# funcwj/setk

Hardware: AMD Instinct MI355X
Metric: real-time-factor (audio-sec/wall-sec), 8-ch 16 kHz MVDR (higher is better)
Workload: dtype f32; 1 GPU; 8-ch 16 kHz oracle-mask MVDR, 30 s utterances, 125 per GPU (BASELINE configs[2] shard: 1000 at 8 GPUs), STFT 512/256/hann/center, inputs resident in HBM; utts_per_gpu=125, channels=8, frames=1876, beamformer=mvdr, parallelism=utterance-sharded x1

## Files before the change

### setk_amd/csrc/mcdft.h

```cpp
#pragma once
#include <hip/hip_runtime.h>
#include <stdint.h>

namespace setk {
namespace mc {

#define MC_DEV __device__ __forceinline__

typedef _Float16 h8 __attribute__((ext_vector_type(8)));
typedef _Float16 h2 __attribute__((ext_vector_type(2)));
typedef float f4 __attribute__((ext_vector_type(4)));
typedef float f2 __attribute__((ext_vector_type(2)));
typedef unsigned u4 __attribute__((ext_vector_type(4)));

enum : int {
    kW_MC_H = 0, kW_MC_L = 4, kW_MS_H = 8, kW_MS_L = 12,
    kW_AR_H = 16, kW_AR_L = 20, kW_AI_H = 24, kW_AI_L = 28,
    kW_TR = 32, kW_TI = 36, kW_TRI = 40,
    kW_OT_H = 44, kW_OT_L = 48,
    kW_BR_H = 52, kW_BR_L = 56, kW_BI_H = 60, kW_BI_L = 64,
    kW_G0_H = 68, kW_G0_L = 72, kW_G1_H = 76, kW_G1_L = 80,
    kW_IT_H = 84, kW_IT_L = 88,
    kTabWords = 92
};

__host__ __device__ constexpr int stage1_n1(int k) {
    return (k % 8 < 4) ? 4 * (k / 8) + k % 8 : 16 + 4 * (k / 8) + k % 8 - 4;
}
__host__ __device__ constexpr int sample_of(int lane, int e) { return 16 * stage1_n1(8 * (lane >> 4) + e) + (lane & 15); }

MC_DEV h8 tab_h8(const unsigned* tab, int word, int lane) {
    u4 w;
    w[0] = tab[(word + 0) * 64 + lane];
    w[1] = tab[(word + 1) * 64 + lane];
    w[2] = tab[(word + 2) * 64 + lane];
    w[3] = tab[(word + 3) * 64 + lane];
    return __builtin_bit_cast(h8, w);
}
MC_DEV float tab_f(const unsigned* tab, int word, int lane) {
    return __builtin_bit_cast(float, tab[word * 64 + lane]);
}

MC_DEV f4 mfma16(h8 a, h8 b, f4 c) { return __builtin_amdgcn_mfma_f32_16x16x32_f16(a, b, c, 0, 0, 0); }

MC_DEV void sub_h2(float a, float b, h2 p, float& la, float& lb) {
    const unsigned w = __builtin_bit_cast(unsigned, p);
    asm("v_fma_mix_f32 %0, %1, 1.0, -%2 op_sel_hi:[0,0,1]" : "=v"(la) : "v"(a), "v"(w));
    asm("v_fma_mix_f32 %0, %1, 1.0, -%2 op_sel:[0,0,1] op_sel_hi:[0,0,1]" : "=v"(lb) : "v"(b), "v"(w));
}

MC_DEV void split8(const float (&v)[8], h8& hi, h8& lo) {
#pragma unroll
    for (int e = 0; e < 8; e += 2) {
        const h2 p = __builtin_convertvector((f2){v[e], v[e + 1]}, h2);
        hi[e] = p[0];
        hi[e + 1] = p[1];
        float la, lb;
        sub_h2(v[e], v[e + 1], p, la, lb);
        const h2 q = __builtin_convertvector((f2){la, lb}, h2);
        lo[e] = q[0];
        lo[e + 1] = q[1];
    }
}
MC_DEV void split8_hi(const float (&v)[8], h8& hi) {
#pragma unroll
    for (int e = 0; e < 8; e += 2) {
        const h2 p = __builtin_convertvector((f2){v[e], v[e + 1]}, h2);
        hi[e] = p[0];
        hi[e + 1] = p[1];
    }
}
MC_DEV void split8_lo(const float (&v)[8], h8 hi, h8& lo) {
#pragma unroll
    for (int e = 0; e < 8; e += 2) {
        float la, lb;
        sub_h2(v[e], v[e + 1], (h2){hi[e], hi[e + 1]}, la, lb);
        const h2 q = __builtin_convertvector((f2){la, lb}, h2);
        lo[e] = q[0];
        lo[e + 1] = q[1];
    }
}
MC_DEV void split8_mul_hi(const float (&v)[8], const float (&w)[8], h8& hi) {
#pragma unroll
    for (int e = 0; e < 8; e += 2) {
        const h2 p = __builtin_convertvector((f2){v[e] * w[e], v[e + 1] * w[e + 1]}, h2);
        hi[e] = p[0];
        hi[e + 1] = p[1];
    }
}
MC_DEV void split8_mul_lo(const float (&v)[8], const float (&w)[8], h8 hi, h8& lo) {
#pragma unroll
    for (int e = 0; e < 8; e += 2) {
        const h2 q = __builtin_convertvector(
            (f2){__builtin_fmaf(v[e], w[e], -(float)hi[e]), __builtin_fmaf(v[e + 1], w[e + 1], -(float)hi[e + 1])}, h2);
        lo[e] = q[0];
        lo[e + 1] = q[1];
    }
}
MC_DEV void split8_mul(const float (&v)[8], const float (&w)[8], h8& hi, h8& lo) {
#pragma unroll
    for (int e = 0; e < 8; e += 2) {
        const h2 p = __builtin_convertvector((f2){v[e] * w[e], v[e + 1] * w[e + 1]}, h2);
        hi[e] = p[0];
        hi[e + 1] = p[1];
        const h2 q = __builtin_convertvector(
            (f2){__builtin_fmaf(v[e], w[e], -(float)p[0]), __builtin_fmaf(v[e + 1], w[e + 1], -(float)p[1])}, h2);
        lo[e] = q[0];
        lo[e + 1] = q[1];
    }
}

MC_DEV f4 mm3_data_a(h8 dh, h8 dl, h8 kh, h8 kl) {
    f4 d = {0.f, 0.f, 0.f, 0.f};
    d = mfma16(dh, kh, d);
    d = mfma16(dl, kh, d);
    d = mfma16(dh, kl, d);
    return d;
}
MC_DEV f4 mm3_data_b(h8 kh, h8 kl, h8 dh, h8 dl) {
    f4 d = {0.f, 0.f, 0.f, 0.f};
    d = mfma16(kh, dh, d);
    d = mfma16(kh, dl, d);
    d = mfma16(kl, dh, d);
    return d;
}

struct Fwd {
    h8 mc_h, mc_l, ms_h, ms_l;
    h8 ar_h, ar_l, ai_h, ai_l;
    float tr[4], ti[4], tri[4];
};
MC_DEV void load_fwd(Fwd& K, const unsigned* tab, int lane) {
    K.mc_h = tab_h8(tab, kW_MC_H, lane);
    K.mc_l = tab_h8(tab, kW_MC_L, lane);
    K.ms_h = tab_h8(tab, kW_MS_H, lane);
    K.ms_l = tab_h8(tab, kW_MS_L, lane);
    K.ar_h = tab_h8(tab, kW_AR_H, lane);
    K.ar_l = tab_h8(tab, kW_AR_L, lane);
    K.ai_h = tab_h8(tab, kW_AI_H, lane);
    K.ai_l = tab_h8(tab, kW_AI_L, lane);
#pragma unroll
    for (int r = 0; r < 4; ++r) {
        K.tr[r] = tab_f(tab, kW_TR + r, lane);
        K.ti[r] = tab_f(tab, kW_TI + r, lane);
        K.tri[r] = tab_f(tab, kW_TRI + r, lane);
    }
}

template <class TileFn>
MC_DEV void forward_t(const float (&x)[8], const float (&w)[8], TileFn tile, const float (&tr)[4],
                      const float (&ti)[4], const float (&tri)[4], f4& zr, f4& zi, f4& a16) {
    h8 xh, xl;
    split8_mul_hi(x, w, xh);
    f4 dc = {0.f, 0.f, 0.f, 0.f}, ds = {0.f, 0.f, 0.f, 0.f};
    {
        const h8 mc_h = tile(0), ms_h = tile(2);
        dc = mfma16(xh, mc_h, dc);
        ds = mfma16(xh, ms_h, ds);
        dc = mfma16(xh, tile(1), dc);
        ds = mfma16(xh, tile(3), ds);
        split8_mul_lo(x, w, xh, xl);
        dc = mfma16(xl, mc_h, dc);
        ds = mfma16(xl, ms_h, ds);
    }
    a16 = ds;
    float b[8];
#pragma unroll
    for (int r = 0; r < 4; ++r) {
        b[r] = fmaf(dc[r], tr[r], -ds[r] * ti[r]);
        b[4 + r] = fmaf(dc[r], ti[r], ds[r] * tri[r]);
    }
    h8 bh, bl;
    split8_hi(b, bh);
    zr = (f4){0.f, 0.f, 0.f, 0.f};
    zi = (f4){0.f, 0.f, 0.f, 0.f};
    {
        const h8 ar_h = tile(4), ai_h = tile(6);
        zr = mfma16(ar_h, bh, zr);
        zi = mfma16(ai_h, bh, zi);
        zr = mfma16(tile(5), bh, zr);
        zi = mfma16(tile(7), bh, zi);
        split8_lo(b, bh, bl);
        zr = mfma16(ar_h, bl, zr);
        zi = mfma16(ai_h, bl, zi);
    }
}
MC_DEV void forward(const float (&x)[8], const float (&w)[8], const Fwd& K, f4& zr, f4& zi, f4& a16) {
    forward_t(x, w, [&](int i) -> h8 {
        switch (i) {
            case 0: return K.mc_h;
            case 1: return K.mc_l;
            case 2: return K.ms_h;
            case 3: return K.ms_l;
            case 4: return K.ar_h;
            case 5: return K.ar_l;
            case 6: return K.ai_h;
            default: return K.ai_l;
        }
    }, K.tr, K.ti, K.tri, zr, zi, a16);
}

MC_DEV int bin_of(int c, int g, int r) { return (g < 2) ? c + 32 * (4 * g + r) : 32 * (13 - 4 * g + r) - c; }
MC_DEV bool bin_valid(int c, int g, int r) { return c != 0 || g < 2 || (g == 2 && r == 3); }

typedef __attribute__((address_space(3))) float* lds_fp;
MC_DEV lds_fp to_lds(float* p) { return (lds_fp)p; }
MC_DEV lds_fp opaque_next(lds_fp p) {
    lds_fp q = p + 1;
    asm volatile("" : "+v"(q));
    return q;
}
MC_DEV void store_bins(lds_fp re, lds_fp im, f4 zr, f4 zi) {
#pragma unroll
    for (int r = 0; r < 4; ++r) re[64 * r] = zr[r];
#pragma unroll
    for (int r = 0; r < 4; ++r) im[64 * r] = zi[r];
}

constexpr int kOddPitch = 20;
MC_DEV void store_a16(float* a16s, int j, int lane, f4 a16) {
    if ((lane & 15) == 0) *reinterpret_cast<f4*>(a16s + j * kOddPitch + (lane >> 4) * 4) = a16;
}
MC_DEV f4 odd_tile(const float* a16s, h8 ot_h, h8 ot_l, int lane, int nrows = 16) {
    const int g = lane >> 4;
    const int j = (lane & 15) < nrows ? (lane & 15) : nrows - 1;
    float v[8];
    const f4 v0 = *reinterpret_cast<const f4*>(a16s + j * kOddPitch + 8 * (g & 1));
    const f4 v1 = *reinterpret_cast<const f4*>(a16s + j * kOddPitch + 8 * (g & 1) + 4);
#pragma unroll
    for (int e = 0; e < 4; ++e) {
        v[e] = v0[e];
        v[4 + e] = v1[e];
    }
    h8 h, l;
    split8(v, h, l);
    const h8 bop = (g < 2) ? h : l;
    f4 d = {0.f, 0.f, 0.f, 0.f};
    d = mfma16(ot_h, bop, d);
    d = mfma16(ot_l, bop, d);
    return d;
}

MC_DEV void stage_tiles(u4* lds, const unsigned* tab, int first_word, int ntiles, int tid, int nthreads) {
    for (int i = tid; i < ntiles * 64; i += nthreads) {
        const int t = i >> 6, l = i & 63;
        u4 w;
#pragma unroll
        for (int k = 0; k < 4; ++k) w[k] = tab[(first_word + 4 * t + k) * 64 + l];
        lds[i] = w;
    }
}
MC_DEV h8 lds_h8(const u4* lds, int tile, int lane) { return __builtin_bit_cast(h8, lds[tile * 64 + lane]); }

struct Inv {
    h8 br_h, br_l, bi_h, bi_l;
    h8 g0_h, g0_l, g1_h, g1_l;
    float tr[4], ti[4];
};
MC_DEV void load_inv(Inv& K, const unsigned* tab, int lane) {
    K.br_h = tab_h8(tab, kW_BR_H, lane);
    K.br_l = tab_h8(tab, kW_BR_L, lane);
    K.bi_h = tab_h8(tab, kW_BI_H, lane);
    K.bi_l = tab_h8(tab, kW_BI_L, lane);
    K.g0_h = tab_h8(tab, kW_G0_H, lane);
    K.g0_l = tab_h8(tab, kW_G0_L, lane);
    K.g1_h = tab_h8(tab, kW_G1_H, lane);
    K.g1_l = tab_h8(tab, kW_G1_L, lane);
#pragma unroll
    for (int r = 0; r < 4; ++r) {
        K.tr[r] = tab_f(tab, kW_TR + r, lane);
        K.ti[r] = tab_f(tab, kW_TI + r, lane);
    }
}

MC_DEV void inverse_a(f4 yr, f4 yi, float e16, h8 br_h, h8 br_l, h8 bi_h, h8 bi_l, const float (&tr)[4],
                      const float (&ti)[4], float (&b)[8], int lane) {
    float a[8];
#pragma unroll
    for (int r = 0; r < 4; ++r) {
        a[r] = yr[r];
        a[4 + r] = yi[r];
    }
    h8 ah, al;
    split8(a, ah, al);
    const f4 cr = mm3_data_a(ah, al, br_h, br_l);
    const f4 ci = mm3_data_a(ah, al, bi_h, bi_l);
#pragma unroll
    for (int r = 0; r < 4; ++r) {
        b[r] = fmaf(cr[r], tr[r], ci[r] * ti[r]);
        b[4 + r] = fmaf(ci[r], tr[r], -cr[r] * ti[r]);
    }
    if (lane < 16) b[4] = e16;
}
MC_DEV void inverse_b(const float (&b)[8], h8 g0_h, h8 g0_l, h8 g1_h, h8 g1_l, f4& y0, f4& y1) {
    h8 bh, bl;
    split8(b, bh, bl);
    y0 = mm3_data_b(g0_h, g0_l, bh, bl);
    y1 = mm3_data_b(g1_h, g1_l, bh, bl);
}
MC_DEV void inverse(f4 yr, f4 yi, float e16, const Inv& K, f4& y0, f4& y1, int lane) {
    float b[8];
    inverse_a(yr, yi, e16, K.br_h, K.br_l, K.bi_h, K.bi_l, K.tr, K.ti, b, lane);
    inverse_b(b, K.g0_h, K.g0_l, K.g1_h, K.g1_l, y0, y1);
}

MC_DEV f4 inv_odd_tile(const float (&v)[8], h8 it_h, h8 it_l, int lane) {
    h8 h, l;
    split8(v, h, l);
    const h8 aop = ((lane >> 4) < 2) ? h : l;
    f4 d = {0.f, 0.f, 0.f, 0.f};
    d = mfma16(aop, it_h, d);
    d = mfma16(aop, it_l, d);
    return d;
}

}
}
```

### setk_amd/csrc/pass2_mc.hip

```cpp
#include "common.h"
#include "fft512.h"
#include "mcdft.h"
#include <cstdio>
#include <cstdlib>
#include <type_traits>

namespace setk {

constexpr int kP2McWavesPerSimd = 4;
constexpr int kP2McGroup = 2;
constexpr int p2mc_threads(bool pcm) { return pcm ? 1024 : 512; }

constexpr int kP2McTiles = 25;
size_t pass2_mc_lds_bytes(int C, bool pcm) {
    const size_t nw = p2mc_threads(pcm) / 64;
    const size_t wt = ((size_t)C * kBins * sizeof(cf) + 15) & ~(size_t)15;
    return wt + kP2McTiles * 1024 + 2048 + nw * kP2McGroup * 8 * mc::kOddPitch * sizeof(float) +
           nw * 16 * sizeof(float) + 64 + (pcm ? nw * C * 64 * sizeof(uint2) : 0);
}

SETK_DEV float row8_sum(float x) {
    int v = __builtin_bit_cast(int, x);
    x += __builtin_bit_cast(float, __builtin_amdgcn_update_dpp(0, v, 0xB1, 0xf, 0xf, true));
    v = __builtin_bit_cast(int, x);
    x += __builtin_bit_cast(float, __builtin_amdgcn_update_dpp(0, v, 0x4E, 0xf, 0xf, true));
    v = __builtin_bit_cast(int, x);
    x += __builtin_bit_cast(float, __builtin_amdgcn_update_dpp(0, v, 0x141, 0xf, 0xf, true));
    return x;
}
SETK_DEV float wave_max_nonneg(float x) {
    int v = __builtin_bit_cast(int, x);
    x = fmaxf(x, __builtin_bit_cast(float, __builtin_amdgcn_update_dpp(0, v, 0xB1, 0xf, 0xf, true)));
    v = __builtin_bit_cast(int, x);
    x = fmaxf(x, __builtin_bit_cast(float, __builtin_amdgcn_update_dpp(0, v, 0x4E, 0xf, 0xf, true)));
    v = __builtin_bit_cast(int, x);
    x = fmaxf(x, __builtin_bit_cast(float, __builtin_amdgcn_update_dpp(0, v, 0x141, 0xf, 0xf, true)));
    v = __builtin_bit_cast(int, x);
    x = fmaxf(x, __builtin_bit_cast(float, __builtin_amdgcn_update_dpp(0, v, 0x140, 0xf, 0xf, true)));
    const unsigned b = __builtin_bit_cast(unsigned, x);
    unsigned m = __builtin_amdgcn_readlane(b, 0);
    const unsigned m1 = __builtin_amdgcn_readlane(b, 16), m2 = __builtin_amdgcn_readlane(b, 32),
                   m3 = __builtin_amdgcn_readlane(b, 48);
    m = m > m1 ? m : m1;
    m = m > m2 ? m : m2;
    m = m > m3 ? m : m3;
    return __builtin_bit_cast(float, m);
}

template <int C, bool PCM = false>
__global__ __launch_bounds__(p2mc_threads(PCM), kP2McWavesPerSimd) void beamform_istft_mc_kernel(Pass2Args a) {
    constexpr int NT = p2mc_threads(PCM);
    constexpr int NW = NT / 64;
    constexpr int F = kBins;

    extern __shared__ __attribute__((aligned(16))) char smem[];
    char* p = smem;
    cf* wtab = reinterpret_cast<cf*>(p);
    p += ((size_t)C * F * sizeof(cf) + 15) & ~(size_t)15;
    mc::u4* tiles = reinterpret_cast<mc::u4*>(p);
    p += kP2McTiles * 1024;
    mc::f4* synr = reinterpret_cast<mc::f4*>(p);
    p += 2048;
    float* a16s = reinterpret_cast<float*>(p);
    p += (size_t)NW * kP2McGroup * 8 * mc::kOddPitch * sizeof(float);
    float* yodd_s = reinterpret_cast<float*>(p);
    p += NW * 16 * sizeof(float);
    float* red = reinterpret_cast<float*>(p);
    p += 64;
    uint2* carry_s = reinterpret_cast<uint2*>(p);

    const int tid = threadIdx.x;
    const int lane = tid & 63;
    const int wave = __builtin_amdgcn_readfirstlane(tid >> 6);
    const int c16 = lane & 15, g = lane >> 4;
    const WorkItem wi = a.items[blockIdx.x];
    const UttDesc ud = a.utts[wi.utt];
    const int n_samp = ud.num_samples;
    const int T = ud.num_frames;
    const int hop = kNfft / 2;
    const bool post_mask = (a.flags & 0x4) != 0;
    const bool clamp = (a.flags & 0x2) != 0;

    float in_sc = PCM ? 3.0517578125e-05f : 1.f, out_sc = 1.f;
    if (a.norm_bits) {
        const unsigned nb = a.norm_bits[wi.utt];
        int e = (int)((nb >> 23) & 0xff) - 126;
        e = (__builtin_bit_cast(float, nb) <= 1.f) ? 0 : (e > 100 ? 100 : e);
        in_sc *= __builtin_bit_cast(float, (unsigned)(127 - e) << 23);
        out_sc = __builtin_bit_cast(float, (unsigned)(127 + e) << 23);
    }
    {
        const cf* wsrc = reinterpret_cast<const cf*>(a.weight) + (size_t)wi.utt * C * kBinsPad;
        for (int i = tid; i < C * F; i += NT) {
            const int c = i / F, f = i - c * F;
            wtab[i] = wsrc[c * kBinsPad + f];
        }
    }
    mc::stage_tiles(tiles, a.mc_tab, mc::kW_BR_H, 10, tid, NT);
    mc::stage_tiles(tiles + 10 * 64, a.mc_tab, mc::kW_OT_H, 2, tid, NT);
    mc::stage_tiles(tiles + 12 * 64, a.mc_tab, mc::kW_MC_H, 8, tid, NT);
    for (int i = tid; i < 128; i += NT) {
        const int l = i & 63, t4 = i >> 6;
        const mc::f4 w = {a.mc_win[(4 * t4 + 0) * 64 + l] * in_sc, a.mc_win[(4 * t4 + 1) * 64 + l] * in_sc,
                          a.mc_win[(4 * t4 + 2) * 64 + l] * in_sc, a.mc_win[(4 * t4 + 3) * 64 + l] * in_sc};
        tiles[20 * 64 + i] = __builtin_bit_cast(mc::u4, w);
    }
    mc::stage_tiles(tiles + 22 * 64, a.mc_tab, mc::kW_TR, 3, tid, NT);
    for (int i = tid; i < 128; i += NT) {
        const int l = i & 63, hf = i >> 6;
        synr[i] = (mc::f4){a.mc_syn[(4 * hf + 0) * 64 + l] * out_sc, a.mc_syn[(4 * hf + 1) * 64 + l] * out_sc,
                           a.mc_syn[(4 * hf + 2) * 64 + l] * out_sc, a.mc_syn[(4 * hf + 3) * 64 + l] * out_sc};
    }
    struct { float tr[4], ti[4]; } K;
    float* yoddw = yodd_s + wave * 16;
    const int lane_bin = mc::bin_of(c16, g, 0);
    const cf* wl = wtab + lane_bin;
    const int jo = c16 < C ? c16 : 0;
    const cf* wo = wtab + jo * F + 16 + 64 * g;
    const bool odd_on = c16 < C;
    const int lane_n = 64 * g + c16;
    float omax = 0.f;
    __syncthreads();

    const int per = (wi.t1 - wi.t0 + NW - 1) / NW;
    const int ta = wi.t0 + wave * per;
    const int tb = min(ta + per, wi.t1);
    const int tw = ta > 0 ? ta - 1 : ta;

    constexpr int R = kP2McGroup;
    float* a16g = a16s + wave * R * 8 * mc::kOddPitch;
    float carry[4] = {0.f, 0.f, 0.f, 0.f};
    auto chan = [&](int c) {
        if constexpr (PCM) return (gcshort_p)gptr(ud.audio) + (size_t)c * ud.ch_stride;
        else return gptr(ud.audio) + (size_t)c * n_samp;
    };
    uint2* carry_l = carry_s + (size_t)wave * C * 64 + lane;
    auto load_full = [&](float (&v)[8], int t, int c, auto edge) __attribute__((always_inline)) {
        if constexpr (PCM) {
            const uint2 pk = carry_l[64 * c];
            v[0] = (float)(short)(pk.x & 0xffff);
            v[1] = (float)((int)pk.x >> 16);
            v[2] = (float)(short)(pk.y & 0xffff);
            v[3] = (float)((int)pk.y >> 16);
            const auto x = chan(c);
            const int s0 = min(t, T - 1) * hop - a.g.pad + 256, o = 64 * g + c16;
            if (!decltype(edge)::value) {
#pragma unroll
                for (int e = 0; e < 4; ++e) v[4 + e] = x[s0 + o + 16 * e];
            } else {
#pragma unroll
                for (int e = 0; e < 4; ++e) v[4 + e] = x[reflect_index(s0 + o + 16 * e, n_samp)];
            }
        } else {
            const auto x = chan(c);
            const int s0 = min(t, T - 1) * hop - a.g.pad, o = 64 * g + c16;
            if (!decltype(edge)::value) {
#pragma unroll
                for (int e = 0; e < 4; ++e) {
                    v[e] = __builtin_nontemporal_load(&x[s0 + o + 16 * e]);
                    v[4 + e] = __builtin_nontemporal_load(&x[s0 + o + 256 + 16 * e]);
                }
            } else {
#pragma unroll
                for (int e = 0; e < 4; ++e) {
                    v[e] = x[reflect_index(s0 + o + 16 * e, n_samp)];
                    v[4 + e] = x[reflect_index(s0 + o + 256 + 16 * e, n_samp)];
                }
            }
        }
    };
    auto load_half_raw = [&](int (&r)[4], int t, int c, auto edge) __attribute__((always_inline)) {
        const auto x = chan(c);
        const int s0 = min(t, T - 1) * hop - a.g.pad + 256, o = 64 * g + c16;
        if (!decltype(edge)::value) {
#pragma unroll
            for (int e = 0; e < 4; ++e) r[e] = x[s0 + o + 16 * e];
        } else {
#pragma unroll
            for (int e = 0; e < 4; ++e) r[e] = x[reflect_index(s0 + o + 16 * e, n_samp)];
        }
    };
    auto load_half = [&](float (&v)[8], int t, int c, auto edge) __attribute__((always_inline)) {
        const auto x = chan(c);
        const int s0 = min(t, T - 1) * hop - a.g.pad + 256, o = 64 * g + c16;
        if (!decltype(edge)::value) {
#pragma unroll
            for (int e = 0; e < 4; ++e) v[4 + e] = x[s0 + o + 16 * e];
        } else {
#pragma unroll
            for (int e = 0; e < 4; ++e) v[4 + e] = x[reflect_index(s0 + o + 16 * e, n_samp)];
        }
    };
    mc::f4 yr[R], yi[R];
    float nxt[8];
    int nraw[4];
    auto group = [&](int t0, auto edge) __attribute__((always_inline)) {
#pragma unroll
        for (int k = 0; k < R; ++k) {
            yr[k] = (mc::f4){0.f, 0.f, 0.f, 0.f};
            yi[k] = (mc::f4){0.f, 0.f, 0.f, 0.f};
        }
#pragma unroll 1
        for (int c = 0; c < C; ++c) {
            asm volatile("" ::: "memory");
            const cf* wc = wl + c * F;
            cf w[4];
#pragma unroll
            for (int r = 0; r < 4; ++r) w[r] = wc[32 * r];
            float x[8];
#pragma unroll
            for (int e = 0; e < 8; ++e) x[e] = nxt[e];
#pragma unroll
            for (int k = 0; k < R; ++k) {
                if (k + 1 < R) {
                    if constexpr (PCM) load_half_raw(nraw, t0 + k + 1, c, edge);
                    else load_half(nxt, t0 + k + 1, c, edge);
                } else if (c + 1 < C) {
                    load_full(nxt, t0, c + 1, edge);
                }
                mc::f4 zr, zi, a16;
                {
                    asm volatile("" ::: "memory");
                    const mc::f4 w0 = __builtin_bit_cast(mc::f4, tiles[20 * 64 + lane]);
                    const mc::f4 w1 = __builtin_bit_cast(mc::f4, tiles[21 * 64 + lane]);
                    const mc::f4 q0 = __builtin_bit_cast(mc::f4, tiles[22 * 64 + lane]);
                    const mc::f4 q1 = __builtin_bit_cast(mc::f4, tiles[23 * 64 + lane]);
                    const mc::f4 q2 = __builtin_bit_cast(mc::f4, tiles[24 * 64 + lane]);
                    const float win[8] = {w0[0], w0[1], w0[2], w0[3], w1[0], w1[1], w1[2], w1[3]};
                    const float tr[4] = {q0[0], q0[1], q0[2], q0[3]}, ti[4] = {q1[0], q1[1], q1[2], q1[3]},
                                tri[4] = {q2[0], q2[1], q2[2], q2[3]};
                    mc::forward_t(x, win, [&](int i) { return mc::lds_h8(tiles, 12 + i, lane); }, tr, ti, tri, zr, zi, a16);
                }
                mc::store_a16(a16g + k * 8 * mc::kOddPitch, c, lane, a16);
#pragma unroll
                for (int r = 0; r < 4; ++r) {
                    yr[k][r] = fmaf(zr[r], w[r].x, fmaf(zi[r], w[r].y, yr[k][r]));
                    yi[k][r] = fmaf(zi[r], w[r].x, fmaf(-zr[r], w[r].y, yi[k][r]));
                }
                if (k + 1 < R) {
#pragma unroll
                    for (int e = 0; e < 4; ++e) {
                        x[e] = x[4 + e];
                        if constexpr (PCM) x[4 + e] = (float)nraw[e];
                        else x[4 + e] = nxt[4 + e];
                    }
                    if constexpr (PCM) {
                        static_assert(R == 2, "the LDS carry is written for groups of two frames");
                        carry_l[64 * c] = make_uint2(__builtin_amdgcn_perm((unsigned)nraw[1], (unsigned)nraw[0], 0x05040100u),
                                                     __builtin_amdgcn_perm((unsigned)nraw[3], (unsigned)nraw[2], 0x05040100u));
                    }
                }
                __builtin_amdgcn_sched_barrier(0);
            }
        }
    };
    auto span_is_edge = [&](int t0) {
        const int lo = t0 * hop - a.g.pad, hi = (t0 + R - 1) * hop - a.g.pad + kNfft;
        return lo < 0 || hi > n_samp || t0 + R > T;
    };
    auto request_group = [&](int t0) __attribute__((always_inline)) {
        if (span_is_edge(t0)) load_full(nxt, t0, 0, std::true_type());
        else load_full(nxt, t0, 0, std::false_type());
    };
    if constexpr (PCM) {
        if (tw < tb) {
#pragma unroll 1
            for (int c = 0; c < C; ++c) {
                const auto x = chan(c);
                const int s0 = tw * hop - a.g.pad, o = 64 * g + c16;
                int r[4];
#pragma unroll
                for (int e = 0; e < 4; ++e) r[e] = x[reflect_index(s0 + o + 16 * e, n_samp)];
                carry_l[64 * c] = make_uint2(__builtin_amdgcn_perm((unsigned)r[1], (unsigned)r[0], 0x05040100u),
                                             __builtin_amdgcn_perm((unsigned)r[3], (unsigned)r[2], 0x05040100u));
            }
        }
    }
    if (tw < tb) request_group(tw);
#pragma unroll 1
    for (int t0 = tw; t0 < tb; t0 += R) {
        const int nf = min(R, tb - t0);
        if (span_is_edge(t0)) group(t0, std::true_type());
        else group(t0, std::false_type());
        if (t0 + R < tb) request_group(t0 + R);
#pragma unroll
        for (int k = 0; k < R; ++k) {
            if (k >= nf) break;
            const int t = t0 + k;
            float yo[4];
            {
                asm volatile("" ::: "memory");
                const mc::f4 d = mc::odd_tile(a16g + k * 8 * mc::kOddPitch, mc::lds_h8(tiles, 10, lane),
                                              mc::lds_h8(tiles, 11, lane), lane, C);
                const cf w0 = wo[0], w1 = wo[32];
                yo[0] = odd_on ? fmaf(d[0], w0.x, d[1] * w0.y) : 0.f;
                yo[1] = odd_on ? fmaf(d[1], w0.x, -d[0] * w0.y) : 0.f;
                yo[2] = odd_on ? fmaf(d[2], w1.x, d[3] * w1.y) : 0.f;
                yo[3] = odd_on ? fmaf(d[3], w1.x, -d[2] * w1.y) : 0.f;
#pragma unroll
                for (int i = 0; i < 4; ++i) yo[i] = row8_sum(yo[i]);
            }
            mc::f4 fr = yr[k], fi = yi[k];
            if (post_mask) {
                const float* mrow = ud.mask_s + (size_t)t * F;
#pragma unroll
                for (int r = 0; r < 4; ++r) {
                    float m = mrow[lane_bin + 32 * r];
                    if (clamp) m = fminf(m, 1.f);
                    fr[r] *= m;
                    fi[r] *= m;
                }
                float m0 = mrow[16 + 64 * g], m1 = mrow[48 + 64 * g];
                if (clamp) { m0 = fminf(m0, 1.f); m1 = fminf(m1, 1.f); }
                yo[0] *= m0;
                yo[1] *= m0;
                yo[2] *= m1;
                yo[3] *= m1;
            }
            fi[0] = (lane == 0) ? 0.f : fi[0];
            fi[3] = (lane == 32) ? 0.f : fi[3];
            float mxl = fmaxf(fmaxf(fabsf(yo[0]), fabsf(yo[1])), fmaxf(fabsf(yo[2]), fabsf(yo[3])));
#pragma unroll
            for (int r = 0; r < 4; ++r) mxl = fmaxf(mxl, fmaxf(fabsf(fr[r]), fabsf(fi[r])));
            const float mxw = wave_max_nonneg(mxl);
            int ex = (int)((__builtin_bit_cast(unsigned, mxw) >> 23) & 0xff);
            ex = ex < 16 ? 16 : (ex > 250 ? 250 : ex);
            const float sc = __builtin_bit_cast(float, (unsigned)(264 - ex) << 23);
            const float isc = __builtin_bit_cast(float, (unsigned)(ex - 10) << 23);
            if (c16 == 0) *reinterpret_cast<mc::f4*>(yoddw + 4 * g) = (mc::f4){yo[0] * sc, yo[1] * sc, yo[2] * sc, yo[3] * sc};
            float e16;
            {
                float v[8];
                const mc::f4 v0 = *reinterpret_cast<const mc::f4*>(yoddw + 8 * (g & 1));
                const mc::f4 v1 = *reinterpret_cast<const mc::f4*>(yoddw + 8 * (g & 1) + 4);
                const float rowsel = c16 == 0 ? 1.f : 0.f;
#pragma unroll
                for (int e = 0; e < 4; ++e) {
                    v[e] = v0[e] * rowsel;
                    v[4 + e] = v1[e] * rowsel;
                }
                const mc::f4 d = mc::inv_odd_tile(v, mc::lds_h8(tiles, 8, lane), mc::lds_h8(tiles, 9, lane), lane);
                e16 = d[0];
            }
#pragma unroll
            for (int r = 0; r < 4; ++r) {
                fr[r] *= sc;
                fi[r] *= sc;
            }
            float bmid[8];
            {
                const mc::f4 tt0 = __builtin_bit_cast(mc::f4, tiles[22 * 64 + lane]);
                const mc::f4 tt1 = __builtin_bit_cast(mc::f4, tiles[23 * 64 + lane]);
#pragma unroll
                for (int r = 0; r < 4; ++r) {
                    K.tr[r] = tt0[r];
                    K.ti[r] = tt1[r];
                }
            }
            mc::inverse_a(fr, fi, e16, mc::lds_h8(tiles, 0, lane), mc::lds_h8(tiles, 1, lane),
                          mc::lds_h8(tiles, 2, lane), mc::lds_h8(tiles, 3, lane), K.tr, K.ti, bmid, lane);
            asm volatile("" ::: "memory");
            mc::f4 y0, y1;
            mc::inverse_b(bmid, mc::lds_h8(tiles, 4, lane), mc::lds_h8(tiles, 5, lane),
                          mc::lds_h8(tiles, 6, lane), mc::lds_h8(tiles, 7, lane), y0, y1);
            const mc::f4 s0 = synr[lane], s1 = synr[64 + lane];
            float blk[4];
#pragma unroll
            for (int r = 0; r < 4; ++r) blk[r] = fmaf(y0[r], s0[r] * isc, carry[r]);
            if (t == 0) {
#pragma unroll
                for (int r = 0; r < 4; ++r) blk[r] *= gptr(a.mc_edge)[r * 64 + lane];
            }
            if (t >= ta) {
                const int o = t * hop - a.g.pad + lane_n;
#pragma unroll
                for (int r = 0; r < 4; ++r) {
                    const int oo = o + 16 * r;
                    if (oo >= 0 && oo < ud.out_len) {
                        ud.wave_f32[oo] = blk[r];
                        omax = fmaxf(omax, fabsf(blk[r]));
                    }
                }
            }
#pragma unroll
            for (int r = 0; r < 4; ++r) carry[r] = y1[r] * (s1[r] * isc);
        }
    }
    if (tb == T && ta < tb) {
        const int o = T * hop - a.g.pad + lane_n;
#pragma unroll
        for (int r = 0; r < 4; ++r) {
            const int oo = o + 16 * r;
            const float v = carry[r] * gptr(a.mc_edge)[(4 + r) * 64 + lane];
            if (oo >= 0 && oo < ud.out_len) {
                ud.wave_f32[oo] = v;
                omax = fmaxf(omax, fabsf(v));
            }
        }
    }
#pragma unroll
    for (int o = 32; o > 0; o >>= 1) omax = fmaxf(omax, __shfl_xor(omax, o));
    if ((tid & 63) == 0) red[tid >> 6] = omax;
    __syncthreads();
    if (tid == 0) {
        float m = red[0];
#pragma unroll
        for (int w = 1; w < NT / 64; ++w) m = fmaxf(m, red[w]);
        atomicMax(a.outmax_bits + wi.utt, __float_as_uint(m));
    }
}

int pass2_mc_wgs_per_cu(int C, bool pcm) {
    const int by_waves = kP2McWavesPerSimd * 4 / (p2mc_threads(pcm) / 64);
    const int by_lds = (int)((160u << 10) / pass2_mc_lds_bytes(C, pcm));
    return by_waves < by_lds ? (by_waves > 0 ? by_waves : 1) : (by_lds > 0 ? by_lds : 1);
}

template <int C, bool PCM = false>
static hipError_t launch_pass2_mc_t(const Pass2Args& a, int n_items, hipStream_t s) {
    const size_t lds = pass2_mc_lds_bytes(C, PCM);
    auto k = beamform_istft_mc_kernel<C, PCM>;
    hipError_t e = hipFuncSetAttribute(reinterpret_cast<const void*>(k),
                                       hipFuncAttributeMaxDynamicSharedMemorySize, (int)lds);
    if (e != hipSuccess) return e;
    hipLaunchKernelGGL(k, dim3(n_items), dim3(p2mc_threads(PCM)), lds, s, a);
    return hipGetLastError();
}

hipError_t launch_pass2_mc(int C, const Pass2Args& a, int n_items, hipStream_t s, bool pcm16) {
#define SETK_CASE(c) \
    case c: return pcm16 ? launch_pass2_mc_t<c, true>(a, n_items, s) : launch_pass2_mc_t<c>(a, n_items, s);
    switch (C) {
        SETK_CASE(1)
        SETK_CASE(2)
        SETK_CASE(3)
        SETK_CASE(4)
        SETK_CASE(5)
        SETK_CASE(6)
        SETK_CASE(7)
        SETK_CASE(8)
    }
#undef SETK_CASE
    return hipErrorInvalidValue;
}

}
```

Before: 2.113 million x real time (audio seconds per wall second, all GPUs).

## Process two frames per pass in MC forward and inverse DFT with shared tile loads

Replaces the per-frame forward and inverse MFMA DFT paths with paired versions that transform two consecutive frames together. Each B/A tile is loaded once from LDS and reused for both frames, and the independent MFMAs are interleaved to hide latency. The odd-bin and inverse stages now handle both frames in one pass, with a doubled yodd scratch buffer in LDS. Input loads for the next channel are merged into a single prefetch. The cost is higher register pressure, which may reduce occupancy at the 4-waves-per-SIMD launch bound.

```diff
diff --git a/setk_amd/csrc/mcdft.h b/setk_amd/csrc/mcdft.h
--- a/setk_amd/csrc/mcdft.h
+++ b/setk_amd/csrc/mcdft.h
@@ -185,6 +185,80 @@
         zi = mfma16(ai_h, bl, zi);
     }
 }
+template <class TileFn, class TwidFn>
+MC_DEV void forward2_t(const float (&x0)[8], const float (&x1)[8], const float (&w)[8], TileFn tile, TwidFn twid,
+                       f4& zr0, f4& zi0, f4& a16_0, f4& zr1, f4& zi1, f4& a16_1) {
+    h8 xh0, xh1, xl0, xl1;
+    split8_mul_hi(x0, w, xh0);
+    split8_mul_hi(x1, w, xh1);
+    f4 dc0 = {0.f, 0.f, 0.f, 0.f}, ds0 = {0.f, 0.f, 0.f, 0.f};
+    f4 dc1 = {0.f, 0.f, 0.f, 0.f}, ds1 = {0.f, 0.f, 0.f, 0.f};
+    {
+        const h8 mc_h = tile(0), ms_h = tile(2);
+        dc0 = mfma16(xh0, mc_h, dc0);
+        dc1 = mfma16(xh1, mc_h, dc1);
+        ds0 = mfma16(xh0, ms_h, ds0);
+        ds1 = mfma16(xh1, ms_h, ds1);
+        {
+            const h8 mc_l = tile(1);
+            dc0 = mfma16(xh0, mc_l, dc0);
+            dc1 = mfma16(xh1, mc_l, dc1);
+        }
+        {
+            const h8 ms_l = tile(3);
+            ds0 = mfma16(xh0, ms_l, ds0);
+            ds1 = mfma16(xh1, ms_l, ds1);
+        }
+        split8_mul_lo(x0, w, xh0, xl0);
+        split8_mul_lo(x1, w, xh1, xl1);
+        dc0 = mfma16(xl0, mc_h, dc0);
+        dc1 = mfma16(xl1, mc_h, dc1);
+        ds0 = mfma16(xl0, ms_h, ds0);
+        ds1 = mfma16(xl1, ms_h, ds1);
+    }
+    a16_0 = ds0;
+    a16_1 = ds1;
+    __builtin_amdgcn_sched_barrier(0);
+    const f4 tr = twid(0), ti = twid(1), tri = twid(2);
+    float b0[8], b1[8];
+#pragma unroll
+    for (int r = 0; r < 4; ++r) {
+        b0[r] = fmaf(dc0[r], tr[r], -ds0[r] * ti[r]);
+        b0[4 + r] = fmaf(dc0[r], ti[r], ds0[r] * tri[r]);
+        b1[r] = fmaf(dc1[r], tr[r], -ds1[r] * ti[r]);
+        b1[4 + r] = fmaf(dc1[r], ti[r], ds1[r] * tri[r]);
+    }
+    h8 bh0, bh1, bl0, bl1;
+    split8_hi(b0, bh0);
+    split8_hi(b1, bh1);
+    zr0 = (f4){0.f, 0.f, 0.f, 0.f};
+    zi0 = (f4){0.f, 0.f, 0.f, 0.f};
+    zr1 = (f4){0.f, 0.f, 0.f, 0.f};
+    zi1 = (f4){0.f, 0.f, 0.f, 0.f};
+    {
+        const h8 ar_h = tile(4), ai_h = tile(6);
+        zr0 = mfma16(ar_h, bh0, zr0);
+        zr1 = mfma16(ar_h, bh1, zr1);
+        zi0 = mfma16(ai_h, bh0, zi0);
+        zi1 = mfma16(ai_h, bh1, zi1);
+        {
+            const h8 ar_l = tile(5);
+            zr0 = mfma16(ar_l, bh0, zr0);
+            zr1 = mfma16(ar_l, bh1, zr1);
+        }
+        {
+            const h8 ai_l = tile(7);
+            zi0 = mfma16(ai_l, bh0, zi0);
+            zi1 = mfma16(ai_l, bh1, zi1);
+        }
+        split8_lo(b0, bh0, bl0);
+        split8_lo(b1, bh1, bl1);
+        zr0 = mfma16(ar_h, bl0, zr0);
+        zr1 = mfma16(ar_h, bl1, zr1);
+        zi0 = mfma16(ai_h, bl0, zi0);
+        zi1 = mfma16(ai_h, bl1, zi1);
+    }
+}
 MC_DEV void forward(const float (&x)[8], const float (&w)[8], const Fwd& K, f4& zr, f4& zi, f4& a16) {
     forward_t(x, w, [&](int i) -> h8 {
         switch (i) {
@@ -221,9 +295,8 @@
 MC_DEV void store_a16(float* a16s, int j, int lane, f4 a16) {
     if ((lane & 15) == 0) *reinterpret_cast<f4*>(a16s + j * kOddPitch + (lane >> 4) * 4) = a16;
 }
-MC_DEV f4 odd_tile(const float* a16s, h8 ot_h, h8 ot_l, int lane, int nrows = 16) {
+MC_DEV f4 odd_tile_row(const float* a16s, h8 ot_h, h8 ot_l, int lane, int j) {
     const int g = lane >> 4;
-    const int j = (lane & 15) < nrows ? (lane & 15) : nrows - 1;
     float v[8];
     const f4 v0 = *reinterpret_cast<const f4*>(a16s + j * kOddPitch + 8 * (g & 1));
     const f4 v1 = *reinterpret_cast<const f4*>(a16s + j * kOddPitch + 8 * (g & 1) + 4);
@@ -239,6 +312,10 @@
     d = mfma16(ot_h, bop, d);
     d = mfma16(ot_l, bop, d);
     return d;
+}
+MC_DEV f4 odd_tile(const float* a16s, h8 ot_h, h8 ot_l, int lane, int nrows = 16) {
+    const int j = (lane & 15) < nrows ? (lane & 15) : nrows - 1;
+    return odd_tile_row(a16s, ot_h, ot_l, lane, j);
 }
 
 MC_DEV void stage_tiles(u4* lds, const unsigned* tab, int first_word, int ntiles, int tid, int nthreads) {
@@ -304,6 +381,93 @@
     inverse_b(b, K.g0_h, K.g0_l, K.g1_h, K.g1_l, y0, y1);
 }
 
+template <class TileFn>
+MC_DEV void inverse2_a(f4 yr0, f4 yi0, float e16_0, f4 yr1, f4 yi1, float e16_1, TileFn tile, const float (&tr)[4],
+                       const float (&ti)[4], float (&b0)[8], float (&b1)[8], int lane) {
+    float a0[8], a1[8];
+#pragma unroll
+    for (int r = 0; r < 4; ++r) {
+        a0[r] = yr0[r];
+        a0[4 + r] = yi0[r];
+        a1[r] = yr1[r];
+        a1[4 + r] = yi1[r];
+    }
+    h8 ah0, al0, ah1, al1;
+    split8(a0, ah0, al0);
+    split8(a1, ah1, al1);
+    f4 cr0 = {0.f, 0.f, 0.f, 0.f}, ci0 = {0.f, 0.f, 0.f, 0.f};
+    f4 cr1 = {0.f, 0.f, 0.f, 0.f}, ci1 = {0.f, 0.f, 0.f, 0.f};
+    {
+        const h8 br_h = tile(0);
+        cr0 = mfma16(ah0, br_h, cr0);
+        cr1 = mfma16(ah1, br_h, cr1);
+        cr0 = mfma16(al0, br_h, cr0);
+        cr1 = mfma16(al1, br_h, cr1);
+    }
+    {
+        const h8 br_l = tile(1);
+        cr0 = mfma16(ah0, br_l, cr0);
+        cr1 = mfma16(ah1, br_l, cr1);
+    }
+    {
+        const h8 bi_h = tile(2);
+        ci0 = mfma16(ah0, bi_h, ci0);
+        ci1 = mfma16(ah1, bi_h, ci1);
+        ci0 = mfma16(al0, bi_h, ci0);
+        ci1 = mfma16(al1, bi_h, ci1);
+    }
+    {
+        const h8 bi_l = tile(3);
+        ci0 = mfma16(ah0, bi_l, ci0);
+        ci1 = mfma16(ah1, bi_l, ci1);
+    }
+#pragma unroll
+    for (int r = 0; r < 4; ++r) {
+        b0[r] = fmaf(cr0[r], tr[r], ci0[r] * ti[r]);
+        b0[4 + r] = fmaf(ci0[r], tr[r], -cr0[r] * ti[r]);
+        b1[r] = fmaf(cr1[r], tr[r], ci1[r] * ti[r]);
+        b1[4 + r] = fmaf(ci1[r], tr[r], -cr1[r] * ti[r]);
+    }
+    if (lane < 16) {
+        b0[4] = e16_0;
+        b1[4] = e16_1;
+    }
+}
+template <class TileFn>
+MC_DEV void inverse2_b(const float (&b0)[8], const float (&b1)[8], TileFn tile, f4& y0_0, f4& y1_0, f4& y0_1, f4& y1_1) {
+    h8 bh0, bl0, bh1, bl1;
+    split8(b0, bh0, bl0);
+    split8(b1, bh1, bl1);
+    y0_0 = (f4){0.f, 0.f, 0.f, 0.f};
+    y1_0 = (f4){0.f, 0.f, 0.f, 0.f};
+    y0_1 = (f4){0.f, 0.f, 0.f, 0.f};
+    y1_1 = (f4){0.f, 0.f, 0.f, 0.f};
+    {
+        const h8 g0_h = tile(4);
+        y0_0 = mfma16(g0_h, bh0, y0_0);
+        y0_1 = mfma16(g0_h, bh1, y0_1);
+        y0_0 = mfma16(g0_h, bl0, y0_0);
+        y0_1 = mfma16(g0_h, bl1, y0_1);
+    }
+    {
+        const h8 g0_l = tile(5);
+        y0_0 = mfma16(g0_l, bh0, y0_0);
+        y0_1 = mfma16(g0_l, bh1, y0_1);
+    }
+    {
+        const h8 g1_h = tile(6);
+        y1_0 = mfma16(g1_h, bh0, y1_0);
+        y1_1 = mfma16(g1_h, bh1, y1_1);
+        y1_0 = mfma16(g1_h, bl0, y1_0);
+        y1_1 = mfma16(g1_h, bl1, y1_1);
+    }
+    {
+        const h8 g1_l = tile(7);
+        y1_0 = mfma16(g1_l, bh0, y1_0);
+        y1_1 = mfma16(g1_l, bh1, y1_1);
+    }
+}
+
 MC_DEV f4 inv_odd_tile(const float (&v)[8], h8 it_h, h8 it_l, int lane) {
     h8 h, l;
     split8(v, h, l);
diff --git a/setk_amd/csrc/pass2_mc.hip b/setk_amd/csrc/pass2_mc.hip
--- a/setk_amd/csrc/pass2_mc.hip
+++ b/setk_amd/csrc/pass2_mc.hip
@@ -16,7 +16,7 @@
     const size_t nw = p2mc_threads(pcm) / 64;
     const size_t wt = ((size_t)C * kBins * sizeof(cf) + 15) & ~(size_t)15;
     return wt + kP2McTiles * 1024 + 2048 + nw * kP2McGroup * 8 * mc::kOddPitch * sizeof(float) +
-           nw * 16 * sizeof(float) + 64 + (pcm ? nw * C * 64 * sizeof(uint2) : 0);
+           nw * kP2McGroup * 16 * sizeof(float) + 64 + (pcm ? nw * C * 64 * sizeof(uint2) : 0);
 }
 
 SETK_DEV float row8_sum(float x) {
@@ -64,7 +64,7 @@
     float* a16s = reinterpret_cast<float*>(p);
     p += (size_t)NW * kP2McGroup * 8 * mc::kOddPitch * sizeof(float);
     float* yodd_s = reinterpret_cast<float*>(p);
-    p += NW * 16 * sizeof(float);
+    p += NW * kP2McGroup * 16 * sizeof(float);
     float* red = reinterpret_cast<float*>(p);
     p += 64;
     uint2* carry_s = reinterpret_cast<uint2*>(p);
@@ -112,12 +112,9 @@
                            a.mc_syn[(4 * hf + 2) * 64 + l] * out_sc, a.mc_syn[(4 * hf + 3) * 64 + l] * out_sc};
     }
     struct { float tr[4], ti[4]; } K;
-    float* yoddw = yodd_s + wave * 16;
+    float* yoddw = yodd_s + wave * kP2McGroup * 16;
     const int lane_bin = mc::bin_of(c16, g, 0);
     const cf* wl = wtab + lane_bin;
-    const int jo = c16 < C ? c16 : 0;
-    const cf* wo = wtab + jo * F + 16 + 64 * g;
-    const bool odd_on = c16 < C;
     const int lane_n = 64 * g + c16;
     float omax = 0.f;
     __syncthreads();
@@ -135,64 +132,51 @@
         else return gptr(ud.audio) + (size_t)c * n_samp;
     };
     uint2* carry_l = carry_s + (size_t)wave * C * 64 + lane;
-    auto load_full = [&](float (&v)[8], int t, int c, auto edge) __attribute__((always_inline)) {
+    auto load_pair = [&](float (&v)[12], int (&nr)[4], int t0, int c, auto edge) __attribute__((always_inline)) {
+        const auto x = chan(c);
+        const int o = 64 * g + c16;
+        const int s0 = min(t0, T - 1) * hop - a.g.pad, s1 = min(t0 + 1, T - 1) * hop - a.g.pad + 256;
         if constexpr (PCM) {
             const uint2 pk = carry_l[64 * c];
             v[0] = (float)(short)(pk.x & 0xffff);
             v[1] = (float)((int)pk.x >> 16);
             v[2] = (float)(short)(pk.y & 0xffff);
             v[3] = (float)((int)pk.y >> 16);
-            const auto x = chan(c);
-            const int s0 = min(t, T - 1) * hop - a.g.pad + 256, o = 64 * g + c16;
             if (!decltype(edge)::value) {
 #pragma unroll
-                for (int e = 0; e < 4; ++e) v[4 + e] = x[s0 + o + 16 * e];
+                for (int e = 0; e < 4; ++e) {
+                    v[4 + e] = x[s0 + o + 256 + 16 * e];
+                    nr[e] = x[s1 + o + 16 * e];
+                }
             } else {
 #pragma unroll
-                for (int e = 0; e < 4; ++e) v[4 + e] = x[reflect_index(s0 + o + 16 * e, n_samp)];
+                for (int e = 0; e < 4; ++e) {
+                    v[4 + e] = x[reflect_index(s0 + o + 256 + 16 * e, n_samp)];
+                    nr[e] = x[reflect_index(s1 + o + 16 * e, n_samp)];
+                }
             }
         } else {
-            const auto x = chan(c);
-            const int s0 = min(t, T - 1) * hop - a.g.pad, o = 64 * g + c16;
             if (!decltype(edge)::value) {
 #pragma unroll
                 for (int e = 0; e < 4; ++e) {
                     v[e] = __builtin_nontemporal_load(&x[s0 + o + 16 * e]);
                     v[4 + e] = __builtin_nontemporal_load(&x[s0 + o + 256 + 16 * e]);
                 }
+#pragma unroll
+                for (int e = 0; e < 4; ++e) v[8 + e] = x[s1 + o + 16 * e];
             } else {
 #pragma unroll
                 for (int e = 0; e < 4; ++e) {
                     v[e] = x[reflect_index(s0 + o + 16 * e, n_samp)];
                     v[4 + e] = x[reflect_index(s0 + o + 256 + 16 * e, n_samp)];
-                }
-            }
-        }
-    };
-    auto load_half_raw = [&](int (&r)[4], int t, int c, auto edge) __attribute__((always_inline)) {
-        const auto x = chan(c);
-        const int s0 = min(t, T - 1) * hop - a.g.pad + 256, o = 64 * g + c16;
-        if (!decltype(edge)::value) {
-#pragma unroll
-            for (int e = 0; e < 4; ++e) r[e] = x[s0 + o + 16 * e];
-        } else {
-#pragma unroll
-            for (int e = 0; e < 4; ++e) r[e] = x[reflect_index(s0 + o + 16 * e, n_samp)];
-        }
-    };
-    auto load_half = [&](float (&v)[8], int t, int c, auto edge) __attribute__((always_inline)) {
-        const auto x = chan(c);
-        const int s0 = min(t, T - 1) * hop - a.g.pad + 256, o = 64 * g + c16;
-        if (!decltype(edge)::value) {
-#pragma unroll
-            for (int e = 0; e < 4; ++e) v[4 + e] = x[s0 + o + 16 * e];
-        } else {
-#pragma unroll
-            for (int e = 0; e < 4; ++e) v[4 + e] = x[reflect_index(s0 + o + 16 * e, n_samp)];
+                    v[8 + e] = x[reflect_index(s1 + o + 16 * e, n_samp)];
+                }
+            }
         }
     };
     mc::f4 yr[R], yi[R];
-    float nxt[8];
+    static_assert(R == 2, "the paired transform and the LDS carry are written for groups of two frames");
+    float nxt[12];
     int nraw[4];
     auto group = [&](int t0, auto edge) __attribute__((always_inline)) {
 #pragma unroll
@@ -202,56 +186,46 @@
         }
 #pragma unroll 1
         for (int c = 0; c < C; ++c) {
+            float x0[8], x1[8];
+#pragma unroll
+            for (int e = 0; e < 4; ++e) {
+                x0[e] = nxt[e];
+                x0[4 + e] = nxt[4 + e];
+                x1[e] = nxt[4 + e];
+                if constexpr (PCM) x1[4 + e] = (float)nraw[e];
+                else x1[4 + e] = nxt[8 + e];
+            }
+            if constexpr (PCM) {
+                carry_l[64 * c] = make_uint2(__builtin_amdgcn_perm((unsigned)nraw[1], (unsigned)nraw[0], 0x05040100u),
+                                             __builtin_amdgcn_perm((unsigned)nraw[3], (unsigned)nraw[2], 0x05040100u));
+            }
+            if (c + 1 < C) load_pair(nxt, nraw, t0, c + 1, edge);
+            mc::f4 zr0, zi0, a16_0, zr1, zi1, a16_1;
+            {
+                asm volatile("" ::: "memory");
+                const mc::f4 w0 = __builtin_bit_cast(mc::f4, tiles[20 * 64 + lane]);
+                const mc::f4 w1 = __builtin_bit_cast(mc::f4, tiles[21 * 64 + lane]);
+                const float win[8] = {w0[0], w0[1], w0[2], w0[3], w1[0], w1[1], w1[2], w1[3]};
+                mc::forward2_t(x0, x1, win, [&](int i) { return mc::lds_h8(tiles, 12 + i, lane); },
+                               [&](int i) { return __builtin_bit_cast(mc::f4, tiles[(22 + i) * 64 + lane]); },
+                               zr0, zi0, a16_0, zr1, zi1, a16_1);
+            }
+            __builtin_amdgcn_sched_barrier(0);
             asm volatile("" ::: "memory");
             const cf* wc = wl + c * F;
             cf w[4];
 #pragma unroll
             for (int r = 0; r < 4; ++r) w[r] = wc[32 * r];
-            float x[8];
-#pragma unroll
-            for (int e = 0; e < 8; ++e) x[e] = nxt[e];
-#pragma unroll
-            for (int k = 0; k < R; ++k) {
-                if (k + 1 < R) {
-                    if constexpr (PCM) load_half_raw(nraw, t0 + k + 1, c, edge);
-                    else load_half(nxt, t0 + k + 1, c, edge);
-                } else if (c + 1 < C) {
-                    load_full(nxt, t0, c + 1, edge);
-                }
-                mc::f4 zr, zi, a16;
-                {
-                    asm volatile("" ::: "memory");
-                    const mc::f4 w0 = __builtin_bit_cast(mc::f4, tiles[20 * 64 + lane]);
-                    const mc::f4 w1 = __builtin_bit_cast(mc::f4, tiles[21 * 64 + lane]);
-                    const mc::f4 q0 = __builtin_bit_cast(mc::f4, tiles[22 * 64 + lane]);
-                    const mc::f4 q1 = __builtin_bit_cast(mc::f4, tiles[23 * 64 + lane]);
-                    const mc::f4 q2 = __builtin_bit_cast(mc::f4, tiles[24 * 64 + lane]);
-                    const float win[8] = {w0[0], w0[1], w0[2], w0[3], w1[0], w1[1], w1[2], w1[3]};
-                    const float tr[4] = {q0[0], q0[1], q0[2], q0[3]}, ti[4] = {q1[0], q1[1], q1[2], q1[3]},
-                                tri[4] = {q2[0], q2[1], q2[2], q2[3]};
-                    mc::forward_t(x, win, [&](int i) { return mc::lds_h8(tiles, 12 + i, lane); }, tr, ti, tri, zr, zi, a16);
-                }
-                mc::store_a16(a16g + k * 8 * mc::kOddPitch, c, lane, a16);
-#pragma unroll
-                for (int r = 0; r < 4; ++r) {
-                    yr[k][r] = fmaf(zr[r], w[r].x, fmaf(zi[r], w[r].y, yr[k][r]));
-                    yi[k][r] = fmaf(zi[r], w[r].x, fmaf(-zr[r], w[r].y, yi[k][r]));
-                }
-                if (k + 1 < R) {
-#pragma unroll
-                    for (int e = 0; e < 4; ++e) {
-                        x[e] = x[4 + e];
-                        if constexpr (PCM) x[4 + e] = (float)nraw[e];
-                        else x[4 + e] = nxt[4 + e];
-                    }
-                    if constexpr (PCM) {
-                        static_assert(R == 2, "the LDS carry is written for groups of two frames");
-                        carry_l[64 * c] = make_uint2(__builtin_amdgcn_perm((unsigned)nraw[1], (unsigned)nraw[0], 0x05040100u),
-                                                     __builtin_amdgcn_perm((unsigned)nraw[3], (unsigned)nraw[2], 0x05040100u));
-                    }
-                }
-                __builtin_amdgcn_sched_barrier(0);
-            }
+            mc::store_a16(a16g, c, lane, a16_0);
+            mc::store_a16(a16g + 8 * mc::kOddPitch, c, lane, a16_1);
+#pragma unroll
+            for (int r = 0; r < 4; ++r) {
+                yr[0][r] = fmaf(zr0[r], w[r].x, fmaf(zi0[r], w[r].y, yr[0][r]));
+                yi[0][r] = fmaf(zi0[r], w[r].x, fmaf(-zr0[r], w[r].y, yi[0][r]));
+                yr[1][r] = fmaf(zr1[r], w[r].x, fmaf(zi1[r], w[r].y, yr[1][r]));
+                yi[1][r] = fmaf(zi1[r], w[r].x, fmaf(-zr1[r], w[r].y, yi[1][r]));
+            }
+            __builtin_amdgcn_sched_barrier(0);
         }
     };
     auto span_is_edge = [&](int t0) {
@@ -259,8 +233,8 @@
         return lo < 0 || hi > n_samp || t0 + R > T;
     };
     auto request_group = [&](int t0) __attribute__((always_inline)) {
-        if (span_is_edge(t0)) load_full(nxt, t0, 0, std::true_type());
-        else load_full(nxt, t0, 0, std::false_type());
+        if (span_is_edge(t0)) load_pair(nxt, nraw, t0, 0, std::true_type());
+        else load_pair(nxt, nraw, t0, 0, std::false_type());
     };
     if constexpr (PCM) {
         if (tw < tb) {
@@ -283,90 +257,118 @@
         if (span_is_edge(t0)) group(t0, std::true_type());
         else group(t0, std::false_type());
         if (t0 + R < tb) request_group(t0 + R);
+        const int t1 = min(t0 + 1, T - 1);
+        int lt = lane;
+        asm volatile("" : "+v"(lt));
+        const int kf = (lt >> 3) & 1, co = lt & 7, c16 = lt & 15, g = lt >> 4;
+        const bool odd_on = co < C;
+        const cf* wo = wtab + (odd_on ? co : 0) * F + 16 + 64 * g;
+        const int orow = 8 * kf + (odd_on ? co : C - 1);
+        float yo[4];
+        {
+            asm volatile("" ::: "memory");
+            const mc::f4 d = mc::odd_tile_row(a16g, mc::lds_h8(tiles, 10, lane), mc::lds_h8(tiles, 11, lane), lane, orow);
+            const cf w0 = wo[0], w1 = wo[32];
+            yo[0] = odd_on ? fmaf(d[0], w0.x, d[1] * w0.y) : 0.f;
+            yo[1] = odd_on ? fmaf(d[1], w0.x, -d[0] * w0.y) : 0.f;
+            yo[2] = odd_on ? fmaf(d[2], w1.x, d[3] * w1.y) : 0.f;
+            yo[3] = odd_on ? fmaf(d[3], w1.x, -d[2] * w1.y) : 0.f;
+#pragma unroll
+            for (int i = 0; i < 4; ++i) yo[i] = row8_sum(yo[i]);
+        }
+        mc::f4 fr[R], fi[R];
+#pragma unroll
+        for (int k = 0; k < R; ++k) {
+            fr[k] = yr[k];
+            fi[k] = yi[k];
+        }
+        if (post_mask) {
+            const float* mrow = ud.mask_s + (size_t)t0 * F;
+            const unsigned dm = (unsigned)(t1 - t0) * F;
+            unsigned mo = (unsigned)lane_bin, mq = 16u + 64u * (unsigned)g + (kf ? dm : 0u);
+            asm volatile("" : "+v"(mo), "+v"(mq));
+#pragma unroll
+            for (int k = 0; k < R; ++k) {
+#pragma unroll
+                for (int r = 0; r < 4; ++r) {
+                    float m = mrow[mo + (k ? dm : 0u) + 32 * r];
+                    if (clamp) m = fminf(m, 1.f);
+                    fr[k][r] *= m;
+                    fi[k][r] *= m;
+                }
+            }
+            float m0 = mrow[mq], m1 = mrow[mq + 32];
+            if (clamp) { m0 = fminf(m0, 1.f); m1 = fminf(m1, 1.f); }
+            yo[0] *= m0;
+            yo[1] *= m0;
+            yo[2] *= m1;
+            yo[3] *= m1;
+        }
+        const float yom = fmaxf(fmaxf(fabsf(yo[0]), fabsf(yo[1])), fmaxf(fabsf(yo[2]), fabsf(yo[3])));
+        float sc[R], isc[R];
+#pragma unroll
+        for (int k = 0; k < R; ++k) {
+            fi[k][0] = (lane == 0) ? 0.f : fi[k][0];
+            fi[k][3] = (lane == 32) ? 0.f : fi[k][3];
+            float mxl = (kf == k) ? yom : 0.f;
+#pragma unroll
+            for (int r = 0; r < 4; ++r) mxl = fmaxf(mxl, fmaxf(fabsf(fr[k][r]), fabsf(fi[k][r])));
+            const float mxw = wave_max_nonneg(mxl);
+            int ex = (int)((__builtin_bit_cast(unsigned, mxw) >> 23) & 0xff);
+            ex = ex < 16 ? 16 : (ex > 250 ? 250 : ex);
+            sc[k] = __builtin_bit_cast(float, (unsigned)(264 - ex) << 23);
+            isc[k] = __builtin_bit_cast(float, (unsigned)(ex - 10) << 23);
+        }
+        {
+            const float scl = kf ? sc[1] : sc[0];
+            if ((c16 & 7) == 0) *reinterpret_cast<mc::f4*>(yoddw + 16 * kf + 4 * g) = (mc::f4){yo[0] * scl, yo[1] * scl, yo[2] * scl, yo[3] * scl};
+        }
+        float e16[R];
+        {
+            float v[8];
+            const mc::f4 v0 = *reinterpret_cast<const mc::f4*>(yoddw + 16 * (c16 & 1) + 8 * (g & 1));
+            const mc::f4 v1 = *reinterpret_cast<const mc::f4*>(yoddw + 16 * (c16 & 1) + 8 * (g & 1) + 4);
+            const float rowsel = c16 < R ? 1.f : 0.f;
+#pragma unroll
+            for (int e = 0; e < 4; ++e) {
+                v[e] = v0[e] * rowsel;
+                v[4 + e] = v1[e] * rowsel;
+            }
+            const mc::f4 d = mc::inv_odd_tile(v, mc::lds_h8(tiles, 8, lane), mc::lds_h8(tiles, 9, lane), lane);
+            e16[0] = d[0];
+            e16[1] = d[1];
+        }
+#pragma unroll
+        for (int k = 0; k < R; ++k) {
+#pragma unroll
+            for (int r = 0; r < 4; ++r) {
+                fr[k][r] *= sc[k];
+                fi[k][r] *= sc[k];
+            }
+        }
+        float bmid0[8], bmid1[8];
+        {
+            const mc::f4 tt0 = __builtin_bit_cast(mc::f4, tiles[22 * 64 + lane]);
+            const mc::f4 tt1 = __builtin_bit_cast(mc::f4, tiles[23 * 64 + lane]);
+#pragma unroll
+            for (int r = 0; r < 4; ++r) {
+                K.tr[r] = tt0[r];
+                K.ti[r] = tt1[r];
+            }
+        }
+        auto inv_tile = [&](int i) { return mc::lds_h8(tiles, i, lane); };
+        mc::inverse2_a(fr[0], fi[0], e16[0], fr[1], fi[1], e16[1], inv_tile, K.tr, K.ti, bmid0, bmid1, lane);
+        asm volatile("" ::: "memory");
+        mc::f4 y0[R], y1[R];
+        mc::inverse2_b(bmid0, bmid1, inv_tile, y0[0], y1[0], y0[1], y1[1]);
+        const mc::f4 s0 = synr[lane], s1 = synr[64 + lane];
 #pragma unroll
         for (int k = 0; k < R; ++k) {
             if (k >= nf) break;
             const int t = t0 + k;
-            float yo[4];
-            {
-                asm volatile("" ::: "memory");
-                const mc::f4 d = mc::odd_tile(a16g + k * 8 * mc::kOddPitch, mc::lds_h8(tiles, 10, lane),
-                                              mc::lds_h8(tiles, 11, lane), lane, C);
-                const cf w0 = wo[0], w1 = wo[32];
-                yo[0] = odd_on ? fmaf(d[0], w0.x, d[1] * w0.y) : 0.f;
-                yo[1] = odd_on ? fmaf(d[1], w0.x, -d[0] * w0.y) : 0.f;
-                yo[2] = odd_on ? fmaf(d[2], w1.x, d[3] * w1.y) : 0.f;
-                yo[3] = odd_on ? fmaf(d[3], w1.x, -d[2] * w1.y) : 0.f;
-#pragma unroll
-                for (int i = 0; i < 4; ++i) yo[i] = row8_sum(yo[i]);
-            }
-            mc::f4 fr = yr[k], fi = yi[k];
-            if (post_mask) {
-                const float* mrow = ud.mask_s + (size_t)t * F;
-#pragma unroll
-                for (int r = 0; r < 4; ++r) {
-                    float m = mrow[lane_bin + 32 * r];
-                    if (clamp) m = fminf(m, 1.f);
-                    fr[r] *= m;
-                    fi[r] *= m;
-                }
-                float m0 = mrow[16 + 64 * g], m1 = mrow[48 + 64 * g];
-                if (clamp) { m0 = fminf(m0, 1.f); m1 = fminf(m1, 1.f); }
-                yo[0] *= m0;
-                yo[1] *= m0;
-                yo[2] *= m1;
-                yo[3] *= m1;
-            }
-            fi[0] = (lane == 0) ? 0.f : fi[0];
-            fi[3] = (lane == 32) ? 0.f : fi[3];
-            float mxl = fmaxf(fmaxf(fabsf(yo[0]), fabsf(yo[1])), fmaxf(fabsf(yo[2]), fabsf(yo[3])));
-#pragma unroll
-            for (int r = 0; r < 4; ++r) mxl = fmaxf(mxl, fmaxf(fabsf(fr[r]), fabsf(fi[r])));
-            const float mxw = wave_max_nonneg(mxl);
-            int ex = (int)((__builtin_bit_cast(unsigned, mxw) >> 23) & 0xff);
-            ex = ex < 16 ? 16 : (ex > 250 ? 250 : ex);
-            const float sc = __builtin_bit_cast(float, (unsigned)(264 - ex) << 23);
-            const float isc = __builtin_bit_cast(float, (unsigned)(ex - 10) << 23);
-            if (c16 == 0) *reinterpret_cast<mc::f4*>(yoddw + 4 * g) = (mc::f4){yo[0] * sc, yo[1] * sc, yo[2] * sc, yo[3] * sc};
-            float e16;
-            {
-                float v[8];
-                const mc::f4 v0 = *reinterpret_cast<const mc::f4*>(yoddw + 8 * (g & 1));
-                const mc::f4 v1 = *reinterpret_cast<const mc::f4*>(yoddw + 8 * (g & 1) + 4);
-                const float rowsel = c16 == 0 ? 1.f : 0.f;
-#pragma unroll
-                for (int e = 0; e < 4; ++e) {
-                    v[e] = v0[e] * rowsel;
-                    v[4 + e] = v1[e] * rowsel;
-                }
-                const mc::f4 d = mc::inv_odd_tile(v, mc::lds_h8(tiles, 8, lane), mc::lds_h8(tiles, 9, lane), lane);
-                e16 = d[0];
-            }
-#pragma unroll
-            for (int r = 0; r < 4; ++r) {
-                fr[r] *= sc;
-                fi[r] *= sc;
-            }
-            float bmid[8];
-            {
-                const mc::f4 tt0 = __builtin_bit_cast(mc::f4, tiles[22 * 64 + lane]);
-                const mc::f4 tt1 = __builtin_bit_cast(mc::f4, tiles[23 * 64 + lane]);
-#pragma unroll
-                for (int r = 0; r < 4; ++r) {
-                    K.tr[r] = tt0[r];
-                    K.ti[r] = tt1[r];
-                }
-            }
-            mc::inverse_a(fr, fi, e16, mc::lds_h8(tiles, 0, lane), mc::lds_h8(tiles, 1, lane),
-                          mc::lds_h8(tiles, 2, lane), mc::lds_h8(tiles, 3, lane), K.tr, K.ti, bmid, lane);
-            asm volatile("" ::: "memory");
-            mc::f4 y0, y1;
-            mc::inverse_b(bmid, mc::lds_h8(tiles, 4, lane), mc::lds_h8(tiles, 5, lane),
-                          mc::lds_h8(tiles, 6, lane), mc::lds_h8(tiles, 7, lane), y0, y1);
-            const mc::f4 s0 = synr[lane], s1 = synr[64 + lane];
             float blk[4];
 #pragma unroll
-            for (int r = 0; r < 4; ++r) blk[r] = fmaf(y0[r], s0[r] * isc, carry[r]);
+            for (int r = 0; r < 4; ++r) blk[r] = fmaf(y0[k][r], s0[r] * isc[k], carry[r]);
             if (t == 0) {
 #pragma unroll
                 for (int r = 0; r < 4; ++r) blk[r] *= gptr(a.mc_edge)[r * 64 + lane];
@@ -383,7 +385,7 @@
                 }
             }
 #pragma unroll
-            for (int r = 0; r < 4; ++r) carry[r] = y1[r] * (s1[r] * isc);
+            for (int r = 0; r < 4; ++r) carry[r] = y1[k][r] * (s1[r] * isc[k]);
         }
     }
     if (tb == T && ta < tb) {
```

Result: faster. 2.158 million x real time (audio seconds per wall second, all GPUs), median of 6 (+2.1%).
